# Symb0x76/ChineseChessZero

Hardware: AMD Instinct MI355X
Metric: self-play MCTS simulations/sec (higher is better)
Workload: dtype u8 rules / f32 Q (reference CPU path) / f64 PUCT (net: fp16)

## Files before the change

chinesechesszero_amd/_lib.py:

```python
from __future__ import annotations

import ctypes as C
import os

import torch

_HERE = os.path.dirname(os.path.abspath(__file__))
LIB_PATH = os.path.join(_HERE, "libcczero.so")

NSQ = 90
SQ_STRIDE = 96
NMOVES = 2086
MAX_LEGAL = 128
MASK_WORDS = 66
PLANES = 10710
REC_BYTES, REC_HDR, REC_IDS, REC_PI = 880, 96, 112, 368
REC_FLAGS, REC_FAST = 103, 1
REC_RESIGNED, REC_PLAYON, REC_VALUE = 2, 4, 8
REC_VALUE_OFF = 92
RESIGN_RESIGNED, RESIGN_PLAYON = 2, 4
HEAD_POL_STRIDE, HEAD_VAL_STRIDE = 1536, 640

ABI_VERSION = 9
CONV_RELU, CONV_DESCENDING, CONV_FORCE_SMALL, CONV_FORCE_TILE, CONV_G16, CONV_G16_EDGE_TILES = 1, 2, 16, 32, 64, 128
# ... 123 lines not shown
    "ccz_legal_moves": (C.c_int, [_P, C.c_int32, _P, _P, _P, _P, _P, _P]),
    "ccz_apply_moves": (C.c_int, [_P, C.c_int32, _P, _P, _P, _P]),
    "ccz_bias_act_f16": (C.c_int, [_P, _P, _P, _P, C.c_int64, C.c_int32]),
    "ccz_conv3x3_c256_f16": (C.c_int, [_P, _P, _P, _P, _P, _P, C.c_int64, C.c_int32]),
    "ccz_conv3x3_stem_f16": (C.c_int, [_P, _P, _P, _P, _P, C.c_int64, C.c_int32]),
    "ccz_pack_live_planes_f16": (C.c_int, [_P, _P, _P, C.c_int32]),
    "ccz_pack_live_planes_rows_f16": (C.c_int, [_P, _P, _P, C.c_int32, _P, _P]),
    "ccz_pack_live_planes_g16_f16": (C.c_int, [_P, _P, _P, C.c_int32, _P, _P]),
    "ccz_pack_conv_weights_g16_f16": (C.c_int, [_P, _P, _P, C.c_int32]),
    "ccz_conv3x3_c256_f16_live": (C.c_int, [_P, _P, _P, _P, _P, _P, C.c_int64, C.c_int32, _P, C.c_int32, C.c_int32]),
    "ccz_conv3x3_stem_f16_live": (C.c_int, [_P, _P, _P, _P, _P, C.c_int64, C.c_int32, _P, C.c_int32, C.c_int32]),
    "ccz_conv3x3_c256_heads_f16": (C.c_int, [_P, _P, _P, _P, _P, _P, _P, _P, _P, C.c_int64, C.c_int32, _P, C.c_int32, C.c_int32]),
    "ccz_heads_conv1x1_f16": (C.c_int, [_P, _P, _P, _P, _P, _P, C.c_int32, C.c_int32, _P]),
    "ccz_fc_f16": (C.c_int, [_P, _P, C.c_int32, _P, _P, _P, C.c_int32, C.c_int32, C.c_int32, C.c_int32, C.c_int32, _P]),
    "ccz_value_out_f32": (C.c_int, [_P, _P, _P, C.c_float, _P, C.c_int32, _P]),
}

_lib = None


def source_hash() -> str | None:
    import glob
    import hashlib
    csrc = os.path.join(_HERE, "csrc")
    files = sorted(glob.glob(os.path.join(csrc, "*.h")) + glob.glob(os.path.join(csrc, "*.hip")), key=os.path.basename)
    files.append(os.path.join(os.path.dirname(_HERE), "include", "cczero.h"))
    if len(files) < 2 or not all(os.path.exists(f) for f in files):
        return None
    h = hashlib.sha256()
    for f in files:
# ... 46 lines not shown
```

chinesechesszero_amd/build.py:

```python
from __future__ import annotations

import os
import subprocess

_HERE = os.path.dirname(os.path.abspath(__file__))


def build(verbose: bool = False) -> str:
    csrc = os.path.join(_HERE, "csrc")
    out = subprocess.run(["make", "-C", csrc], capture_output=True, text=True)
    if verbose or out.returncode != 0:
        print(out.stdout)
        print(out.stderr)
    if out.returncode != 0:
        raise RuntimeError("hipcc build of libcczero.so failed")
    path = os.path.join(_HERE, "libcczero.so")
    if not os.path.exists(path):
        raise RuntimeError("libcczero.so was not produced")
    return path


_HASHED = ("csrc/*.h", "csrc/*.hip", "csrc/Makefile", "engine.py", "selfplay.py", "net.py", "_lib.py", "replay.py", "../include/cczero.h", "../bench.py")


def code_hash() -> str:
# ... 10 lines not shown
```

chinesechesszero_amd/csrc/cczero.hip:

```cpp
#include "../../include/cczero.h"

#include <hip/hip_runtime.h>

#include <cmath>
#include <cstdarg>
#include <cstdio>
#include <cstring>
#include <new>
#include <vector>

#include "cczero_kernels.h"
#include "cczero_netops.h"
#include "cczero_conv.h"
#include "cczero_conv_small.h"
#include "cczero_conv_g16.h"
#include "cczero_conv_g16e.h"
#include "cczero_heads.h"

using namespace ccz;

namespace {

thread_local char g_err[512] = "";

// ... 37 lines not shown
    std::vector<void *> owned;
    size_t bytes = 0;
    int32_t *st_k = nullptr, *st_visits = nullptr, *st_rootn = nullptr;
    uint16_t *st_acts = nullptr;
    float *st_q = nullptr, *st_p = nullptr;
    double *st_pi = nullptr, *st_temps = nullptr;
    double *st_g = nullptr, *st_u = nullptr;
    long long *st_rowbase = nullptr;
    uint8_t *st_mask = nullptr, *st_sq = nullptr;
    std::vector<BoardMeta> h_meta;
    int active = 0;
    bool routed = false;
    uint8_t *route_red = nullptr;
    uint8_t *route_net = nullptr;
    uint64_t salt[2] = {0, 0};
    bool budgets_on = false;
    bool explore_on = false;
    uint8_t *proof = nullptr, *st_proof = nullptr;
    bool solver_on = false;
};

#define ACTIVE(e) ((unsigned)((e)->active > 0 ? (e)->active : (e)->d.B))

template <typename T> static int fetch_board_stats(ccz_engine *e, hipStream_t s, const T *dev, std::vector<T> &st)
{
    st.resize((size_t)e->d.B);
    HIP_TRY(hipMemcpyAsync(st.data(), dev, st.size() * sizeof(T), hipMemcpyDeviceToHost, s));
    HIP_TRY(hipStreamSynchronize(s));
    return 0;
}
// ... 151 lines not shown
    d.cache = nullptr;
    d.cache_mask = 0;
    if (cfg->eval_cache_log2) {
        const size_t slots = (size_t)1 << cfg->eval_cache_log2;
        d.cache_mask = (uint32_t)(slots - 1);
        ALLOC(d.cache, slots);
        ALLOC(d.claim, slots);
        ALLOC(d.cslot, B);
        ALLOC(d.ctag, B);
        ALLOC(d.cstate, B);
        ALLOC(d.cins, B);
        ALLOC(d.cver, B);
        ALLOC(d.crep, B);
        ALLOC(d.row_of, B);
        ALLOC(d.vleaf, B);
        if (he == hipSuccess) he = hipMemset(d.claim, 0x7f, slots * 4);
    }
    ALLOC(d.rec_sq, B * d.max_plies * 96);
    ALLOC(d.rec_turn, B * d.max_plies);
    ALLOC(d.rec_k, B * d.max_plies);
    ALLOC(d.rec_off, B * d.max_plies);
    ALLOC(d.rec_target, B * d.max_plies);
    ALLOC(d.budget, B);
    ALLOC(d.move_sims, B);
    ALLOC(d.target, B);
    ResignCfg *rs_cfg = nullptr;
    ALLOC(rs_cfg, 1);
    d.rs_cfg = rs_cfg;
    ALLOC(d.rs_state, B);
    ALLOC(d.rs_run, B * 2);
// ... 179 lines not shown
    hipStream_t s = (hipStream_t)stream;
    if (logits_f16)
        hipLaunchKernelGGL((k_softmax_gather<_Float16, false>), dim3(e->d.B), dim3(64), 0, s, e->d, (const _Float16 *)logits_dev, (const float *)nullptr);
    else
        hipLaunchKernelGGL((k_softmax_gather<float, false>), dim3(e->d.B), dim3(64), 0, s, e->d, (const float *)logits_dev, (const float *)nullptr);
    HIP_TRY(hipGetLastError());
    return 0;
}

int ccz_eval_plan(ccz_engine *e, void *stream, int32_t *miss_rows_dev, int32_t *n_miss_dev)
{
    NEED(e);
    if (!e->d.cache) return fail(-1, "ccz_eval_plan: the engine was created without an evaluation cache (ccz_config.eval_cache_log2)");
    if (!miss_rows_dev || !n_miss_dev) return fail(-1, "ccz_eval_plan: null output");
    hipStream_t s = (hipStream_t)stream;
    hipLaunchKernelGGL(k_cache_probe, dim3(e->d.B), dim3(64), 0, s, e->d);
    HIP_TRY(hipGetLastError());
    hipLaunchKernelGGL(k_cache_plan, dim3(1), dim3(1024), 0, s, e->d, miss_rows_dev, n_miss_dev);
    HIP_TRY(hipGetLastError());
    return 0;
}

int ccz_set_scouts(ccz_engine *e, int32_t n_scouts)
{
    NEED(e);
    if (n_scouts < 0 || n_scouts >= e->d.B) return fail(-1, "ccz_set_scouts: n_scouts must be in 0 .. n_boards - 1 (got %d of %d boards)", n_scouts, e->d.B);
    if (n_scouts && !e->d.cache) return fail(-1, "ccz_set_scouts: scouts work through the evaluation cache (ccz_config.eval_cache_log2)");
    if (n_scouts && e->budgets_on) return fail(-1, "ccz_set_scouts: not while simulation budgets are on (ccz_set_budgets(NULL) turns them off)");
    if (n_scouts && e->explore_on) return fail(-1, "ccz_set_scouts: not while root exploration is on (ccz_set_root_exploration)");
    e->active = n_scouts ? e->d.B - n_scouts : 0;
    return 0;
}

// ... 1044 lines not shown
    HIP_TRY(hipGetLastError());
    return 0;
}

int ccz_value_out_f32(void *stream, const void *h_dev, const void *w2_dev, float b2, float *v_dev, int32_t m, const int32_t *live_rows_dev)
{
    if (!h_dev || !w2_dev || !v_dev || m < 0) return fail(-1, "ccz_value_out_f32: bad arguments");
    if ((((uintptr_t)h_dev) | ((uintptr_t)w2_dev)) & 7) return fail(-1, "ccz_value_out_f32: h and w2 must be 8-byte aligned");
    if (m == 0) return 0;
    hipLaunchKernelGGL(k_value_out, dim3((unsigned)((m + 3) / 4)), dim3(256), 0, (hipStream_t)stream, (const _Float16 *)h_dev, (const _Float16 *)w2_dev, b2, v_dev,
                       (int)m, (const int *)live_rows_dev);
    HIP_TRY(hipGetLastError());
    return 0;
}

}
```

chinesechesszero_amd/csrc/cczero_heads.h:

```cpp
#pragma once
#include <hip/hip_runtime.h>
#include <stdint.h>

#include "cczero_conv.h"
#include "cczero_device.h"

namespace ccz {

constexpr int kHdPol = 17, kHdVal = 7;
constexpr int kHdPolStride = 1536;
constexpr int kHdValStride = 640;

template <bool G16>
__global__ __launch_bounds__(256) void k_head_conv1x1(const _Float16 *__restrict__ X, const _Float16 *__restrict__ Wh,
                                                        const float *__restrict__ bh, _Float16 *__restrict__ pol,
                                                        _Float16 *__restrict__ val, int n_boards, const int *__restrict__ live)
{
    const int lane = threadIdx.x & 63, r = lane & 15, q4 = lane >> 4;
    const int wave = blockIdx.x * 4 + (threadIdx.x >> 6), n_waves = gridDim.x * 4;
    int nb = n_boards;
    if (live) { const int l = *live; nb = l < nb ? l : nb; }
    const long n_rows = G16 ? (long)((nb + 15) >> 4) * 1440 : (long)nb * 90;
    const int n_cells = (int)((n_rows + 15) >> 4);
    if (wave >= n_cells) return;
// ... 55 lines not shown
            for (int s = 0; s < 8; ++s) b[s] = bn[s];
        }
    }
}

constexpr int kFcBM = 128, kFcBN = 128, kFcBK = 32, kFcStages = 4;
constexpr int kFcTile = 128 * kFcBK * 2;
constexpr int kFcStage = 2 * kFcTile;
constexpr int kFcERow = 144;
static_assert(4 * 64 * kFcERow <= kFcStages * kFcStage, "the epilogue blocks live in the operand ring");
#ifdef CCZ_FC_DIAG
#define FC_DBG(bit) (dbg & (bit))
#else
#define FC_DBG(bit) 0
#endif
template <bool RELU>
__global__ __launch_bounds__(256) void k_fc_f16(const _Float16 *__restrict__ A, int lda, const _Float16 *__restrict__ W,
                                                  const float *__restrict__ bias, _Float16 *__restrict__ C, int ldc, int M, int N,
                                                  int K, const int *__restrict__ live, [[maybe_unused]] int dbg)
{
    __shared__ __attribute__((aligned(16))) unsigned char lds[kFcStages * kFcStage];
    const int tid = threadIdx.x, lane = tid & 63, r = lane & 15, q4 = lane >> 4;
    const int wv = __builtin_amdgcn_readfirstlane(tid >> 6), wn = wv & 1, wm = wv >> 1;
    int Ml = M;
    if (live) { const int l = *live; Ml = l < Ml ? l : Ml; }
    const int mt = (Ml + kFcBM - 1) / kFcBM, nt = (N + kFcBN - 1) / kFcBN, tiles = mt * nt;
    int n0, m0;
    {
        const int b = blockIdx.x, x = b & 7, per = tiles >> 3, rem = tiles & 7;
        if ((b >> 3) >= per + (x < rem ? 1 : 0)) return;
        const int t = x * per + (x < rem ? x : rem) + (b >> 3);
        const int full = (mt >> 2) * 4 * nt;
        const int blk = t < full ? t / (4 * nt) : (mt >> 2);
        const int r_ = t < full ? t % (4 * nt) : t - full;
        const int cnt = t < full ? 4 : mt - 4 * blk;
        n0 = (r_ / cnt) * kFcBN;
        m0 = (4 * blk + r_ % cnt) * kFcBM;
    }
    const _Float16 *wsrc[2], *asrc[2];
    int wdst[2];
#pragma unroll
    for (int j = 0; j < 2; ++j) {
        const int row = (j * 4 + wv) * 16 + (lane >> 2), c = (lane & 3) ^ ((lane >> 4) & 3);
        wsrc[j] = W + (long)(n0 + row) * K + c * 8;
        int m = m0 + row;
        m = m < Ml ? m : Ml - 1;
        asrc[j] = A + (long)m * lda + c * 8;
        wdst[j] = (j * 4 + wv) * 1024;
    }
    auto issue = [&](int kt) {
        unsigned char *st = lds + (kt & (kFcStages - 1)) * kFcStage;
        const int k0 = kt * kFcBK;
        cv_glds16(wsrc[0] + k0, st + wdst[0]);
        cv_glds16(wsrc[1] + k0, st + wdst[1]);
        cv_glds16(asrc[0] + k0, st + kFcTile + wdst[0]);
        cv_glds16(asrc[1] + k0, st + kFcTile + wdst[1]);
    };
    cv_f32x4 acc[4][4];
#pragma unroll
    for (int i = 0; i < 4; ++i) {
        const float4 bv = *(const float4 *)(bias + n0 + wn * 64 + i * 16 + 4 * q4);
#pragma unroll
        for (int j = 0; j < 4; ++j) { acc[i][j][0] = bv.x; acc[i][j][1] = bv.y; acc[i][j][2] = bv.z; acc[i][j][3] = bv.w; }
    }
    const int nk = K / kFcBK;
    issue(0);
    if (nk > 1) issue(1);
    if (nk > 2) issue(2);
    const int foff = r * 64 + ((q4 ^ ((r >> 2) & 3)) << 4);
    for (int kt = 0; kt < nk; ++kt) {
        if (kt + 2 < nk) cv_wait_vm<8>();
        else if (kt + 1 < nk) cv_wait_vm<4>();
        else cv_wait_vm<0>();
        __builtin_amdgcn_sched_barrier(0);
        if (!FC_DBG(16)) __builtin_amdgcn_s_barrier();
        __builtin_amdgcn_sched_barrier(0);
        if (kt + 3 < nk && !FC_DBG(4)) issue(kt + 3);
        const unsigned char *wb = lds + (kt & (kFcStages - 1)) * kFcStage + wn * 4096 + foff;
        const unsigned char *ab = lds + (kt & (kFcStages - 1)) * kFcStage + kFcTile + wm * 4096 + foff;
        cv_half8 fa[4], fb[4];
        if (!FC_DBG(2) || kt == 0) {
#pragma unroll
            for (int i = 0; i < 4; ++i) fa[i] = *(const cv_half8 *)(wb + i * 1024);
#pragma unroll
            for (int j = 0; j < 4; ++j) fb[j] = *(const cv_half8 *)(ab + j * 1024);
        }
        if (!FC_DBG(1)) {
#pragma unroll
            for (int i = 0; i < 4; ++i)
#pragma unroll
                for (int j = 0; j < 4; ++j) acc[i][j] = __builtin_amdgcn_mfma_f32_16x16x32_f16(fa[i], fb[j], acc[i][j], 0, 0, 0);
        } else {
#pragma unroll
            for (int i = 0; i < 4; ++i) acc[i][0] += (cv_f32x4){(float)fa[i][0], (float)fb[i][0], 0.0f, 0.0f};
        }
    }
    if (FC_DBG(8)) { if (acc[0][0][0] == 12345.678f) C[0] = (_Float16)1; return; }
    __builtin_amdgcn_sched_barrier(0);
    __builtin_amdgcn_s_barrier();
    __builtin_amdgcn_sched_barrier(0);
    {
        unsigned char *tb = lds + wv * (64 * kFcERow);
#pragma unroll
        for (int j = 0; j < 4; ++j)
#pragma unroll
            for (int i = 0; i < 4; ++i) {
                float v0 = acc[i][j][0], v1 = acc[i][j][1], v2 = acc[i][j][2], v3 = acc[i][j][3];
                if (RELU) { v0 = fmaxf(v0, 0.0f); v1 = fmaxf(v1, 0.0f); v2 = fmaxf(v2, 0.0f); v3 = fmaxf(v3, 0.0f); }
                cv_half4 o;
                o[0] = (_Float16)v0; o[1] = (_Float16)v1; o[2] = (_Float16)v2; o[3] = (_Float16)v3;
                *(cv_half4 *)(tb + (j * 16 + r) * kFcERow + (i * 16 + 4 * q4) * 2) = o;
// ... 183 lines not shown
        }
    wave_sync();
    constexpr int NW = NF * 8;
#pragma unroll 4
    for (int it = 0; it < NW; ++it) {
        const int L = it * 64 + lane, row = L / NW, dw = L - row * NW;
        const int m = m0 + wm * 64 + row, n = n0 + I0 * 16 + 2 * dw;
        const uint32_t v = *(const uint32_t *)(tb + row * kFwERow + dw * 4);
        if (m < Ml && n + 1 < N) *(uint32_t *)(C + (long)m * ldc + n) = v;
    }
    FW_STAMP(3)
#undef FW_STAMP
}

template <bool RELU>
__global__ __launch_bounds__(512) void k_fc_wide_f16(const _Float16 *__restrict__ A, int lda, const _Float16 *__restrict__ W,
                                                       const float *__restrict__ bias, _Float16 *__restrict__ C, int ldc, int M, int N,
                                                       int K, const int *__restrict__ live, [[maybe_unused]] int dbg)
{
    __shared__ __attribute__((aligned(16))) unsigned char lds[kFwStages * kFwStage];
    const int tid = threadIdx.x, lane = tid & 63;
    const int wv = __builtin_amdgcn_readfirstlane(tid >> 6), wm = wv & 3, wn = wv >> 2;
    int Ml = M;
    if (live) { const int l = *live; Ml = l < Ml ? l : Ml; }
    const int mt = (Ml + kFwBM - 1) / kFwBM, nt = (N + kFwBN - 1) / kFwBN, tiles = mt * nt;
    int n0, m0;
    {
        const int b = blockIdx.x, x = b & 7, per = tiles >> 3, rem = tiles & 7;
        if ((b >> 3) >= per + (x < rem ? 1 : 0)) return;
        const int t = x * per + (x < rem ? x : rem) + (b >> 3);
        const int full = (mt >> 1) * 2 * nt;
        const int blk = t < full ? t / (2 * nt) : (mt >> 1);
        const int r_ = t < full ? t % (2 * nt) : t - full;
        const int cnt = t < full ? 2 : 1;
        n0 = (r_ / cnt) * kFwBN;
        m0 = (2 * blk + r_ % cnt) * kFwBM;
    }
    const int wrows = ((N + 127) >> 7) << 7;
    const int c = (lane & 7) ^ ((4 * (wv & 1) + (lane >> 4)) & 7), lr = lane >> 3;
    const _Float16 *src[7];
#pragma unroll
    for (int t = 0; t < 4; ++t) {
        int m = m0 + (wv + 8 * t) * 8 + lr;
        m = m < Ml ? m : Ml - 1;
        src[t] = A + (long)m * lda + c * 8;
    }
#pragma unroll
    for (int t = 0; t < 3; ++t) {
        int n = n0 + (wv + 8 * t) * 8 + lr;
        n = n < wrows ? n : wrows - 1;
        src[4 + t] = W + (long)n * K + c * 8;
    }
    if (wn == 0) fw_wave<RELU, 5, 0>(lds, src, wv, wm, lane, bias, wrows - 4, C, ldc, Ml, N, K, m0, n0, dbg);
    else fw_wave<RELU, 4, 5>(lds, src, wv, wm, lane, bias, wrows - 4, C, ldc, Ml, N, K, m0, n0, dbg);
}

__global__ __launch_bounds__(256) void k_value_out(const _Float16 *__restrict__ h, const _Float16 *__restrict__ w2, float b2,
                                                    float *__restrict__ v, int M, const int *__restrict__ live)
{
    const int lane = threadIdx.x & 63, m = blockIdx.x * 4 + (threadIdx.x >> 6);
    if (m >= M) return;
    const cv_half4 x = *(const cv_half4 *)(h + (long)m * 256 + lane * 4), w = *(const cv_half4 *)(w2 + lane * 4);
    int Ml = M;
    if (live) { const int l = *live; Ml = l < Ml ? l : Ml; }
    if (m >= Ml) return;
    float s = (float)x[0] * (float)w[0];
    s += (float)x[1] * (float)w[1];
    s += (float)x[2] * (float)w[2];
    s += (float)x[3] * (float)w[3];
    s = wave_sum_f32(s) + b2;
    if (lane == 0) v[m] = tanhf((float)(_Float16)s);
}

}
```

chinesechesszero_amd/csrc/cczero_kernels.h:

```cpp
#pragma once
#include <type_traits>

#include "cczero_device.h"

namespace ccz {

constexpr uint16_t kHalfOne = 0x3C00;
constexpr int kMaxDepth = 512;

__device__ __forceinline__ void set_err(const Dev &D, int bit) { atomicOr(D.err, bit); }

__device__ __forceinline__ int start_piece(int s)
{
    const int r = s / 9, f = s - 9 * r;
    const int rr = r <= 4 ? r : 9 - r;
    const int add = r <= 4 ? 0 : 8;
    int t = 0;
    if (rr == 0) {
        const int ff = f <= 4 ? f : 8 - f;
        t = ff == 0 ? ROOK : ff == 1 ? KNIGHT : ff == 2 ? BISHOP : ff == 3 ? ADVISOR : KING;
    } else if (rr == 2) {
        t = (f == 1 || f == 7) ? CANNON : 0;
    } else if (rr == 3) {
        t = (f & 1) ? 0 : PAWN;
// ... 1027 lines not shown
        }
    }
    if (tid == 0) {
        n_miss[0] = s_base[0];
        if (ROUTED) n_miss[1] = s_base[1];
    }
}

__global__ __launch_bounds__(1024) void k_cache_plan(Dev D, int32_t *miss_rows, int32_t *n_miss)
{
    __shared__ int s_wave[2][16];
    __shared__ int s_base[2];
    cache_plan_block<false>(D, miss_rows, n_miss, nullptr, 0ull, 0ull, s_wave, s_base);
}

__global__ __launch_bounds__(1024) void k_cache_plan_routed(Dev D, int32_t *miss_rows, int32_t *n_miss, const uint8_t *net, uint64_t salt0,
                                                            uint64_t salt1)
{
    __shared__ int s_wave[2][16];
    __shared__ int s_base[2];
    cache_plan_block<true>(D, miss_rows, n_miss, net, salt0, salt1, s_wave, s_base);
}

__device__ inline void plan_scouted_block(const Dev &D, int active, int32_t *miss_rows, int32_t *n_miss, int32_t *state_out, int tid, int nt, int &s_any)
{
    if (tid == 0) s_any = 0;
    __syncthreads();
    for (int b = tid; b < D.B; b += nt) {
        const int st = D.cstate[b];
        if (b < active) {
// ... 1180 lines not shown
```

chinesechesszero_amd/net.py:

```python
from __future__ import annotations

import ctypes as C
import os

import numpy as np
import torch
import torch.nn.functional as F
from torch import nn

PIECES = 7
PLAYS = 17


class ResBlock(nn.Module):

    def __init__(self, num_channels=256):
        super().__init__()
        self.conv1 = nn.Conv2d(num_channels, num_channels, kernel_size=(3, 3), stride=(1, 1), padding=1)
        self.conv1_bn = nn.BatchNorm2d(num_channels)
        self.conv1_act = nn.ReLU()
        self.conv2 = nn.Conv2d(num_channels, num_channels, kernel_size=(3, 3), stride=(1, 1), padding=1)
        self.conv2_bn = nn.BatchNorm2d(num_channels)
        self.conv2_act = nn.ReLU()

# ... 468 lines not shown
                         torch.zeros((Bx, _lib.HEAD_VAL_STRIDE), dtype=torch.float16, device=dev),
                         torch.empty((Bx, 256), dtype=torch.float16, device=dev))
        return bufs[key]

    def _heads_fused(self, x, B, g16, plan, conv_done=False):
        from . import _lib
        L = _lib.lib()
        Bx, dev = x.shape[0], x.device
        pol, val, h1 = self._head_buffers(Bx, dev)
        logits = torch.empty((B, 2086), dtype=torch.float16, device=dev)
        v = torch.empty((B,), dtype=torch.float32, device=dev)
        s = C.c_void_p(torch.cuda.current_stream(dev).cuda_stream)
        live = _ptr(plan[1]) if plan is not None else None
        if not conv_done:
            _lib.check(L.ccz_heads_conv1x1_f16(s, _ptr(x), _ptr(self.head_w32), _ptr(self.head_b32), _ptr(pol), _ptr(val), Bx, _lib.CONV_G16 if g16 else 0, live))
        _lib.check(L.ccz_fc_f16(s, _ptr(pol), _lib.HEAD_POL_STRIDE, _ptr(self.policy_fc_wp), _ptr(self.policy_fc_b32), _ptr(logits), 2086, B, 2086, 1536, 0, live))
        _lib.check(L.ccz_fc_f16(s, _ptr(val), _lib.HEAD_VAL_STRIDE, _ptr(self.value_fc1_wp), _ptr(self.value_fc1_b32), _ptr(h1), 256, B, 256, 640, 1, live))
        _lib.check(L.ccz_value_out_f32(s, _ptr(h1), _ptr(self.value_fc2_w), self._value_b2(), _ptr(v), B, live))
        return logits, v

    def _value_b2(self) -> float:
        b2 = self.__dict__.get("_b2")
        if b2 is None:
            b2 = self.__dict__["_b2"] = float(self.value_fc2_b.detach().float().cpu().item())
        return b2

    def _heads(self, x, B, g16, plan, return_logits, conv_done=False):
        if self._fused_heads_ok(x):
            logits, v = self._heads_fused(x, B, g16, plan, conv_done)
            if return_logits:
# ... 151 lines not shown
```

include/cczero.h:

```cpp
#ifndef CCZERO_H
#define CCZERO_H

#include <stdint.h>

#ifdef __cplusplus
extern "C" {
#endif

#define CCZ_ABI_VERSION 9
#define CCZ_NSQ 90
#define CCZ_SQ_STRIDE 96
#define CCZ_NMOVES 2086
#define CCZ_MAX_LEGAL 128
#define CCZ_MASK_WORDS 66
#define CCZ_PLANES 10710


#define CCZ_RULE_PAWN_MOVE_RESETS_CLOCK 2u
#define CCZ_RULE_PERPETUAL_CHECK 1u

#define CCZ_FLAG_REFERENCE_QUIRKS 1u
#define CCZ_FLAG_NO_MIRROR 2u
#define CCZ_FLAG_VALUE_F16 4u

// ... 232 lines not shown
                              const void *residual_dev, void *y_dev, int64_t n_pixels, int32_t relu,
                              const int32_t *live_rows_dev, int32_t part, int32_t n_parts);
int ccz_conv3x3_stem_f16_live(void *stream, const void *x64_dev, const void *w_dev, const void *bias_f32_dev,
                              void *y_dev, int64_t n_pixels, int32_t relu, const int32_t *live_rows_dev,
                              int32_t part, int32_t n_parts);

#define CCZ_HEAD_POL_STRIDE 1536
#define CCZ_HEAD_VAL_STRIDE 640
int ccz_heads_conv1x1_f16(void *stream, const void *x_dev, const void *w32_dev, const void *bias32_f32_dev, void *pol_dev,
                          void *val_dev, int32_t n_boards, int32_t flags, const int32_t *live_boards_dev);
int ccz_fc_f16(void *stream, const void *a_dev, int32_t lda, const void *w_dev, const void *bias_f32_dev, void *c_dev, int32_t ldc,
               int32_t m, int32_t n, int32_t k, int32_t relu, const int32_t *live_rows_dev);
int ccz_value_out_f32(void *stream, const void *h_dev, const void *w2_dev, float b2, float *v_dev, int32_t m,
                      const int32_t *live_rows_dev);

int ccz_conv3x3_c256_heads_f16(void *stream, const void *x_dev, const void *w_dev, const void *bias_f32_dev,
                               const void *residual_dev, const void *head_w32_dev, const void *head_bias32_f32_dev,
                               void *pol_dev, void *val_dev, int64_t n_pixels, int32_t flags,
                               const int32_t *live_rows_dev, int32_t part, int32_t n_parts);

#ifdef __cplusplus
}
#endif
#endif
```

profiles/summarize.py:

```python
#!/usr/bin/env python3
import csv
import glob
import json
import os
import sys
from collections import defaultdict


def find(d, pat):
    r = sorted(glob.glob(os.path.join(d, "**", pat), recursive=True))
    return r[0] if r else None


def main():
    out_dir, tag = sys.argv[1], sys.argv[2]
    root = os.path.dirname(os.path.abspath(__file__))
    summary = {}
    prev = os.path.join(root, f"{tag}_summary.json")
    if os.path.exists(prev):
        with open(prev) as f:
            summary = json.load(f)
    stats = find(os.path.join(out_dir, "trace"), "*kernel_stats.csv")
    if stats:
        rows = list(csv.DictReader(open(stats)))
        keep = rows[:48] + [r for r in rows[48:] if "ccz" in r.get("Name", "")]
        with open(os.path.join(root, f"{tag}_kernel_stats.csv"), "w", newline="") as f:
            w = csv.DictWriter(f, fieldnames=list(rows[0].keys()))
            w.writeheader()
            w.writerows(keep)
        for k in ("k_step", "k_softmax_gather", "k_select", "k_expand_backup", "k_finish_move", "k_harvest", "k_bias_act", "k_conv3x3"):
            hit = [r for r in rows if k in r.get("Name", "")]
            if hit:
                calls = sum(int(float(r.get("Calls", 0) or 0)) for r in hit)
                tot = sum(float(r.get("TotalDurationNs", 0) or 0) for r in hit)
                summary.setdefault(k, {})["avg_ns"] = tot / max(1, calls)
                summary[k]["calls"] = calls
                summary[k]["pct"] = sum(float(r.get("Percentage", 0) or 0) for r in hit)
                if len(hit) > 1:
                    summary[k]["variants"] = {r["Name"][:80]: {"calls": int(float(r["Calls"])), "avg_ns": float(r["AverageNs"])} for r in hit}
        plan_calls = sum(int(float(r.get("Calls", 0) or 0)) for r in rows if "k_cache_plan" in r.get("Name", ""))
        if plan_calls:
            tail = {}
            for k in ("k_cache_probe", "k_cache_plan", "k_pack_live_planes", "k_head_conv1x1", "k_fc_f16", "k_fc_wide_f16", "k_value_out", "k_softmax_gather"):
                tot = sum(float(r.get("TotalDurationNs", 0) or 0) for r in rows if k in r.get("Name", ""))
                calls = sum(int(float(r.get("Calls", 0) or 0)) for r in rows if k in r.get("Name", ""))
                if calls:
                    tail[k] = {"us_per_step": tot / plan_calls * 1e-3, "launches_per_step": calls / plan_calls, "avg_us": tot / calls * 1e-3}
            def fam(pred):
                hit = [r for r in rows if pred(r.get("Name", ""))]
                calls = sum(int(float(r.get("Calls", 0) or 0)) for r in hit)
                tot = sum(float(r.get("TotalDurationNs", 0) or 0) for r in hit)
                return calls, tot
            extra, detail = 0.0, {}
            for name, heads, plain in (("middle", lambda n: "k_conv3x3_g16_heads" in n, lambda n: "k_conv3x3_g16<true>" in n or "k_conv3x3_g16ILb1" in n),
                                       ("edge", lambda n: "k_conv3x3_g16_edge_heads" in n, lambda n: "k_conv3x3_g16_edge<true>" in n or "k_conv3x3_g16_edgeILb1" in n)):
                hc, ht = fam(heads)
                pc, pt = fam(plain)
                if hc and pc:
# ... 3 lines not shown
            if detail:
                tail["heads_in_last_tower_layer"] = {"us_per_step": extra, "launches_per_step": sum(v["launches_per_step"] for v in detail.values()),
                                                     "avg_us": extra / max(1e-9, sum(v["launches_per_step"] for v in detail.values())), "detail": detail,
                                                     "what": "launch time of the last layer with the heads in its epilogue minus an ordinary residual layer's, x launches per step "
                                                             "(the chains run concurrently: an upper bound on what the step pays)"}
            other = [(r.get("Name", ""), float(r.get("TotalDurationNs", 0) or 0), int(float(r.get("Calls", 0) or 0))) for r in rows
                     if "ccz" not in r.get("Name", "")]
            summary["evaluator_tail"] = {"kernels": tail, "us_per_step_ours": sum(v["us_per_step"] for v in tail.values()),
                                         "library_kernels_total_us_per_step": sum(t for _, t, _ in other) / plan_calls * 1e-3,
                                         "library_kernels_top": [{"name": n[:90], "us_per_step": t / plan_calls * 1e-3, "calls": c} for n, t, c in sorted(other, key=lambda x: -x[1])[:8]],
                                         "steps": plan_calls,
                                         "what": "non-tower evaluator work per lockstep step (rocprofv3 --kernel-trace --stats of bench.py --steps 120): cache probe + plan, "
                                                 "pack of the live planes, head convolutions, FC layers, value head, softmax + gather + cache store. "
                                                 "library_kernels_*: kernels that are not this library's (torch elementwise / GEMM / copies), whole run "
                                                 "(set-up, preroll and the CPU-side bookkeeping included) divided by the number of steps"}
    def bench_line(name):
        p = os.path.join(out_dir, name)
        if not os.path.exists(p):
            return None
        try:
            return json.loads([l for l in open(p).read().splitlines() if l.startswith("{")][-1])
        except Exception:
            return None

    both_here = all(find(os.path.join(out_dir, k), "*counter_collection.csv") for k in ("pmc_fetch", "pmc_write"))
    if both_here:
        for key in ("k_bar", "d_bar", "warning"):
            summary.get("k_step", {}).get("window", {}).pop(key, None)
    for kind, counter in (("pmc_fetch", "FETCH_SIZE"), ("pmc_write", "WRITE_SIZE"), ("pmc_cfetch", "FETCH_SIZE"), ("pmc_cwrite", "WRITE_SIZE"),
                          ("pmc_hfetch", "FETCH_SIZE"), ("pmc_hwrite", "WRITE_SIZE")):
# ... 112 lines not shown
```

Before: 200,000.

## Fuse cache probe and plan into one launch; fuse policy and value FC heads

Replaces the two-kernel cache probe plus single-block plan with one kernel that probes across many blocks and lets the last block to finish, detected through an atomic ticket, run the plan. It also adds a combined heads kernel for large batches: some workgroups compute the policy FC tile and others compute value FC1, ReLU and the value output using shared LDS. This removes launches and serialization at the step boundary. In exchange it adds the complexity of a last-block ticket and a heterogeneous grid.

```diff
diff --git a/chinesechesszero_amd/_lib.py b/chinesechesszero_amd/_lib.py
--- a/chinesechesszero_amd/_lib.py
+++ b/chinesechesszero_amd/_lib.py
@@ -161,6 +161,7 @@
     "ccz_heads_conv1x1_f16": (C.c_int, [_P, _P, _P, _P, _P, _P, C.c_int32, C.c_int32, _P]),
     "ccz_fc_f16": (C.c_int, [_P, _P, C.c_int32, _P, _P, _P, C.c_int32, C.c_int32, C.c_int32, C.c_int32, C.c_int32, _P]),
     "ccz_value_out_f32": (C.c_int, [_P, _P, _P, C.c_float, _P, C.c_int32, _P]),
+    "ccz_heads_fc_f16": (C.c_int, [_P, _P, _P, _P, _P, C.c_int32, _P, _P, _P, _P, C.c_float, _P, _P, C.c_int32, _P]),
 }
 
 _lib = None
diff --git a/chinesechesszero_amd/build.py b/chinesechesszero_amd/build.py
--- a/chinesechesszero_amd/build.py
+++ b/chinesechesszero_amd/build.py
@@ -8,7 +8,7 @@
 
 def build(verbose: bool = False) -> str:
     csrc = os.path.join(_HERE, "csrc")
-    out = subprocess.run(["make", "-C", csrc], capture_output=True, text=True)
+    out = subprocess.run(["make", "-j2", "-C", csrc, "all", "twolaunch"], capture_output=True, text=True)
     if verbose or out.returncode != 0:
         print(out.stdout)
         print(out.stderr)
diff --git a/chinesechesszero_amd/csrc/cczero.hip b/chinesechesszero_amd/csrc/cczero.hip
--- a/chinesechesszero_amd/csrc/cczero.hip
+++ b/chinesechesszero_amd/csrc/cczero.hip
@@ -75,6 +75,7 @@
     uint8_t *route_red = nullptr;
     uint8_t *route_net = nullptr;
     uint64_t salt[2] = {0, 0};
+    uint32_t *plan_ticket = nullptr;
     bool budgets_on = false;
     bool explore_on = false;
     uint8_t *proof = nullptr, *st_proof = nullptr;
@@ -256,6 +257,7 @@
         ALLOC(d.crep, B);
         ALLOC(d.row_of, B);
         ALLOC(d.vleaf, B);
+        ALLOC(e->plan_ticket, 1);
         if (he == hipSuccess) he = hipMemset(d.claim, 0x7f, slots * 4);
     }
     ALLOC(d.rec_sq, B * d.max_plies * 96);
@@ -465,9 +467,13 @@
     if (!e->d.cache) return fail(-1, "ccz_eval_plan: the engine was created without an evaluation cache (ccz_config.eval_cache_log2)");
     if (!miss_rows_dev || !n_miss_dev) return fail(-1, "ccz_eval_plan: null output");
     hipStream_t s = (hipStream_t)stream;
+#ifdef CCZ_EVAL_PLAN_TWO_LAUNCH
     hipLaunchKernelGGL(k_cache_probe, dim3(e->d.B), dim3(64), 0, s, e->d);
     HIP_TRY(hipGetLastError());
     hipLaunchKernelGGL(k_cache_plan, dim3(1), dim3(1024), 0, s, e->d, miss_rows_dev, n_miss_dev);
+#else
+    hipLaunchKernelGGL(k_eval_plan, dim3((unsigned)((e->d.B + kPlanWaves - 1) / kPlanWaves)), dim3(64 * kPlanWaves), 0, s, e->d, miss_rows_dev, n_miss_dev, e->plan_ticket);
+#endif
     HIP_TRY(hipGetLastError());
     return 0;
 }
@@ -1542,4 +1548,23 @@
     return 0;
 }
 
-}
+int ccz_heads_fc_f16(void *stream, const void *pol_dev, const void *wp_dev, const void *bp_f32_dev, void *logits_dev, int32_t ldc, const void *val_dev,
+                     const void *w1_dev, const void *b1_f32_dev, const void *w2_dev, float b2, float *v_dev, void *h1_dev, int32_t m, const int32_t *live_rows_dev)
+{
+    constexpr int n = 2086;
+    if (!pol_dev || !wp_dev || !bp_f32_dev || !logits_dev || !val_dev || !w1_dev || !b1_f32_dev || !w2_dev || !v_dev || m < 0) return fail(-1, "ccz_heads_fc_f16: bad arguments");
+    if ((ldc & 1) || ldc < n) return fail(-1, "ccz_heads_fc_f16: ldc must be even and >= %d", n);
+    if ((((uintptr_t)pol_dev) | ((uintptr_t)wp_dev) | ((uintptr_t)bp_f32_dev) | ((uintptr_t)val_dev) | ((uintptr_t)w1_dev) | ((uintptr_t)b1_f32_dev)) & 15 ||
+        ((uintptr_t)logits_dev & 3) || ((uintptr_t)w2_dev & 7) || ((uintptr_t)v_dev & 3) || ((uintptr_t)h1_dev & 7))
+        return fail(-1, "ccz_heads_fc_f16: pol, val, the FC weights and biases must be 16-byte aligned, w2 and h1 8-byte, logits and v 4-byte aligned");
+    if (m == 0) return 0;
+    const int wtiles = ((n + kFwBN - 1) / kFwBN) * ((m + kFwBM - 1) / kFwBM);
+    const int pol_blocks = 8 * ((wtiles + 7) / 8), val_blocks = (m + kHvTiles * kFcBM - 1) / (kHvTiles * kFcBM);
+    hipLaunchKernelGGL(k_heads_fc_f16, dim3((unsigned)(pol_blocks + val_blocks)), dim3(512), 0, (hipStream_t)stream, (const _Float16 *)pol_dev, (const _Float16 *)wp_dev,
+                       (const float *)bp_f32_dev, (_Float16 *)logits_dev, (int)ldc, n, (const _Float16 *)val_dev, (const _Float16 *)w1_dev, (const float *)b1_f32_dev,
+                       (const _Float16 *)w2_dev, b2, v_dev, (_Float16 *)h1_dev, (int)m, (const int *)live_rows_dev, pol_blocks, (int)kHdPolStride);
+    HIP_TRY(hipGetLastError());
+    return 0;
+}
+
+}
diff --git a/chinesechesszero_amd/csrc/cczero_heads.h b/chinesechesszero_amd/csrc/cczero_heads.h
--- a/chinesechesszero_amd/csrc/cczero_heads.h
+++ b/chinesechesszero_amd/csrc/cczero_heads.h
@@ -93,6 +93,70 @@
 #else
 #define FC_DBG(bit) 0
 #endif
+__device__ __forceinline__ void fc_tile_acc(unsigned char *lds, const _Float16 *__restrict__ A, int lda, const _Float16 *__restrict__ W,
+                                            const float *__restrict__ bias, int Ml, int K, int m0, int n0, int wv, int lane,
+                                            cv_f32x4 (&acc)[4][4], [[maybe_unused]] int dbg)
+{
+    const int r = lane & 15, q4 = lane >> 4, wn = wv & 1, wm = wv >> 1;
+    const _Float16 *wsrc[2], *asrc[2];
+    int wdst[2];
+#pragma unroll
+    for (int j = 0; j < 2; ++j) {
+        const int row = (j * 4 + wv) * 16 + (lane >> 2), c = (lane & 3) ^ ((lane >> 4) & 3);
+        wsrc[j] = W + (long)(n0 + row) * K + c * 8;
+        int m = m0 + row;
+        m = m < Ml ? m : Ml - 1;
+        asrc[j] = A + (long)m * lda + c * 8;
+        wdst[j] = (j * 4 + wv) * 1024;
+    }
+    auto issue = [&](int kt) {
+        unsigned char *st = lds + (kt & (kFcStages - 1)) * kFcStage;
+        const int k0 = kt * kFcBK;
+        cv_glds16(wsrc[0] + k0, st + wdst[0]);
+        cv_glds16(wsrc[1] + k0, st + wdst[1]);
+        cv_glds16(asrc[0] + k0, st + kFcTile + wdst[0]);
+        cv_glds16(asrc[1] + k0, st + kFcTile + wdst[1]);
+    };
+#pragma unroll
+    for (int i = 0; i < 4; ++i) {
+        const float4 bv = *(const float4 *)(bias + n0 + wn * 64 + i * 16 + 4 * q4);
+#pragma unroll
+        for (int j = 0; j < 4; ++j) { acc[i][j][0] = bv.x; acc[i][j][1] = bv.y; acc[i][j][2] = bv.z; acc[i][j][3] = bv.w; }
+    }
+    const int nk = K / kFcBK;
+    issue(0);
+    if (nk > 1) issue(1);
+    if (nk > 2) issue(2);
+    const int foff = r * 64 + ((q4 ^ ((r >> 2) & 3)) << 4);
+    for (int kt = 0; kt < nk; ++kt) {
+        if (kt + 2 < nk) cv_wait_vm<8>();
+        else if (kt + 1 < nk) cv_wait_vm<4>();
+        else cv_wait_vm<0>();
+        __builtin_amdgcn_sched_barrier(0);
+        if (!FC_DBG(16)) __builtin_amdgcn_s_barrier();
+        __builtin_amdgcn_sched_barrier(0);
+        if (kt + 3 < nk && !FC_DBG(4)) issue(kt + 3);
+        const unsigned char *wb = lds + (kt & (kFcStages - 1)) * kFcStage + wn * 4096 + foff;
+        const unsigned char *ab = lds + (kt & (kFcStages - 1)) * kFcStage + kFcTile + wm * 4096 + foff;
+        cv_half8 fa[4], fb[4];
+        if (!FC_DBG(2) || kt == 0) {
+#pragma unroll
+            for (int i = 0; i < 4; ++i) fa[i] = *(const cv_half8 *)(wb + i * 1024);
+#pragma unroll
+            for (int j = 0; j < 4; ++j) fb[j] = *(const cv_half8 *)(ab + j * 1024);
+        }
+        if (!FC_DBG(1)) {
+#pragma unroll
+            for (int i = 0; i < 4; ++i)
+#pragma unroll
+                for (int j = 0; j < 4; ++j) acc[i][j] = __builtin_amdgcn_mfma_f32_16x16x32_f16(fa[i], fb[j], acc[i][j], 0, 0, 0);
+        } else {
+#pragma unroll
+            for (int i = 0; i < 4; ++i) acc[i][0] += (cv_f32x4){(float)fa[i][0], (float)fb[i][0], 0.0f, 0.0f};
+        }
+    }
+}
+
 template <bool RELU>
 __global__ __launch_bounds__(256) void k_fc_f16(const _Float16 *__restrict__ A, int lda, const _Float16 *__restrict__ W,
                                                   const float *__restrict__ bias, _Float16 *__restrict__ C, int ldc, int M, int N,
@@ -116,64 +180,8 @@
         n0 = (r_ / cnt) * kFcBN;
         m0 = (4 * blk + r_ % cnt) * kFcBM;
     }
-    const _Float16 *wsrc[2], *asrc[2];
-    int wdst[2];
-#pragma unroll
-    for (int j = 0; j < 2; ++j) {
-        const int row = (j * 4 + wv) * 16 + (lane >> 2), c = (lane & 3) ^ ((lane >> 4) & 3);
-        wsrc[j] = W + (long)(n0 + row) * K + c * 8;
-        int m = m0 + row;
-        m = m < Ml ? m : Ml - 1;
-        asrc[j] = A + (long)m * lda + c * 8;
-        wdst[j] = (j * 4 + wv) * 1024;
-    }
-    auto issue = [&](int kt) {
-        unsigned char *st = lds + (kt & (kFcStages - 1)) * kFcStage;
-        const int k0 = kt * kFcBK;
-        cv_glds16(wsrc[0] + k0, st + wdst[0]);
-        cv_glds16(wsrc[1] + k0, st + wdst[1]);
-        cv_glds16(asrc[0] + k0, st + kFcTile + wdst[0]);
-        cv_glds16(asrc[1] + k0, st + kFcTile + wdst[1]);
-    };
     cv_f32x4 acc[4][4];
-#pragma unroll
-    for (int i = 0; i < 4; ++i) {
-        const float4 bv = *(const float4 *)(bias + n0 + wn * 64 + i * 16 + 4 * q4);
-#pragma unroll
-        for (int j = 0; j < 4; ++j) { acc[i][j][0] = bv.x; acc[i][j][1] = bv.y; acc[i][j][2] = bv.z; acc[i][j][3] = bv.w; }
-    }
-    const int nk = K / kFcBK;
-    issue(0);
-    if (nk > 1) issue(1);
-    if (nk > 2) issue(2);
-    const int foff = r * 64 + ((q4 ^ ((r >> 2) & 3)) << 4);
-    for (int kt = 0; kt < nk; ++kt) {
-        if (kt + 2 < nk) cv_wait_vm<8>();
-        else if (kt + 1 < nk) cv_wait_vm<4>();
-        else cv_wait_vm<0>();
-        __builtin_amdgcn_sched_barrier(0);
-        if (!FC_DBG(16)) __builtin_amdgcn_s_barrier();
-        __builtin_amdgcn_sched_barrier(0);
-        if (kt + 3 < nk && !FC_DBG(4)) issue(kt + 3);
-        const unsigned char *wb = lds + (kt & (kFcStages - 1)) * kFcStage + wn * 4096 + foff;
-        const unsigned char *ab = lds + (kt & (kFcStages - 1)) * kFcStage + kFcTile + wm * 4096 + foff;
-        cv_half8 fa[4], fb[4];
-        if (!FC_DBG(2) || kt == 0) {
-#pragma unroll
-            for (int i = 0; i < 4; ++i) fa[i] = *(const cv_half8 *)(wb + i * 1024);
-#pragma unroll
-            for (int j = 0; j < 4; ++j) fb[j] = *(const cv_half8 *)(ab + j * 1024);
-        }
-        if (!FC_DBG(1)) {
-#pragma unroll
-            for (int i = 0; i < 4; ++i)
-#pragma unroll
-                for (int j = 0; j < 4; ++j) acc[i][j] = __builtin_amdgcn_mfma_f32_16x16x32_f16(fa[i], fb[j], acc[i][j], 0, 0, 0);
-        } else {
-#pragma unroll
-            for (int i = 0; i < 4; ++i) acc[i][0] += (cv_f32x4){(float)fa[i][0], (float)fb[i][0], 0.0f, 0.0f};
-        }
-    }
+    fc_tile_acc(lds, A, lda, W, bias, Ml, K, m0, n0, wv, lane, acc, dbg);
     if (FC_DBG(8)) { if (acc[0][0][0] == 12345.678f) C[0] = (_Float16)1; return; }
     __builtin_amdgcn_sched_barrier(0);
     __builtin_amdgcn_s_barrier();
@@ -387,19 +395,16 @@
 }
 
 template <bool RELU>
-__global__ __launch_bounds__(512) void k_fc_wide_f16(const _Float16 *__restrict__ A, int lda, const _Float16 *__restrict__ W,
-                                                       const float *__restrict__ bias, _Float16 *__restrict__ C, int ldc, int M, int N,
-                                                       int K, const int *__restrict__ live, [[maybe_unused]] int dbg)
-{
-    __shared__ __attribute__((aligned(16))) unsigned char lds[kFwStages * kFwStage];
+__device__ __forceinline__ void fw_block(unsigned char *lds, int b, const _Float16 *__restrict__ A, int lda, const _Float16 *__restrict__ W,
+                                         const float *__restrict__ bias, _Float16 *__restrict__ C, int ldc, int Ml, int N, int K,
+                                         [[maybe_unused]] int dbg)
+{
     const int tid = threadIdx.x, lane = tid & 63;
     const int wv = __builtin_amdgcn_readfirstlane(tid >> 6), wm = wv & 3, wn = wv >> 2;
-    int Ml = M;
-    if (live) { const int l = *live; Ml = l < Ml ? l : Ml; }
     const int mt = (Ml + kFwBM - 1) / kFwBM, nt = (N + kFwBN - 1) / kFwBN, tiles = mt * nt;
     int n0, m0;
     {
-        const int b = blockIdx.x, x = b & 7, per = tiles >> 3, rem = tiles & 7;
+        const int x = b & 7, per = tiles >> 3, rem = tiles & 7;
         if ((b >> 3) >= per + (x < rem ? 1 : 0)) return;
         const int t = x * per + (x < rem ? x : rem) + (b >> 3);
         const int full = (mt >> 1) * 2 * nt;
@@ -428,6 +433,27 @@
     else fw_wave<RELU, 4, 5>(lds, src, wv, wm, lane, bias, wrows - 4, C, ldc, Ml, N, K, m0, n0, dbg);
 }
 
+template <bool RELU>
+__global__ __launch_bounds__(512) void k_fc_wide_f16(const _Float16 *__restrict__ A, int lda, const _Float16 *__restrict__ W,
+                                                       const float *__restrict__ bias, _Float16 *__restrict__ C, int ldc, int M, int N,
+                                                       int K, const int *__restrict__ live, [[maybe_unused]] int dbg)
+{
+    __shared__ __attribute__((aligned(16))) unsigned char lds[kFwStages * kFwStage];
+    int Ml = M;
+    if (live) { const int l = *live; Ml = l < Ml ? l : Ml; }
+    fw_block<RELU>(lds, blockIdx.x, A, lda, W, bias, C, ldc, Ml, N, K, dbg);
+}
+
+__device__ __forceinline__ float value_out_wave(cv_half4 x, cv_half4 w, float b2)
+{
+    float s = (float)x[0] * (float)w[0];
+    s += (float)x[1] * (float)w[1];
+    s += (float)x[2] * (float)w[2];
+    s += (float)x[3] * (float)w[3];
+    s = wave_sum_f32(s) + b2;
+    return tanhf((float)(_Float16)s);
+}
+
 __global__ __launch_bounds__(256) void k_value_out(const _Float16 *__restrict__ h, const _Float16 *__restrict__ w2, float b2,
                                                     float *__restrict__ v, int M, const int *__restrict__ live)
 {
@@ -437,12 +463,62 @@
     int Ml = M;
     if (live) { const int l = *live; Ml = l < Ml ? l : Ml; }
     if (m >= Ml) return;
-    float s = (float)x[0] * (float)w[0];
-    s += (float)x[1] * (float)w[1];
-    s += (float)x[2] * (float)w[2];
-    s += (float)x[3] * (float)w[3];
-    s = wave_sum_f32(s) + b2;
-    if (lane == 0) v[m] = tanhf((float)(_Float16)s);
-}
-
-}
+    const float t = value_out_wave(x, w, b2);
+    if (lane == 0) v[m] = t;
+}
+
+constexpr int kHvK = 640, kHvHidden = 256;
+constexpr int kHvHRow = kHvHidden * 2 + 16;
+constexpr int kHvTiles = 2;
+static_assert(2 * kFcStages * kFcStage <= kFwStages * kFwStage && kFcBM * kHvHRow <= kFwStages * kFwStage, "the value workgroup lives in the policy tile's LDS");
+
+__device__ __forceinline__ void hv_block(unsigned char *lds, int vb, const _Float16 *__restrict__ A, const _Float16 *__restrict__ W1,
+                                         const float *__restrict__ b1, const _Float16 *__restrict__ w2, float b2, float *__restrict__ v, _Float16 *__restrict__ h1, int Ml)
+{
+    const int tid = threadIdx.x, lane = tid & 63, r = lane & 15, q4 = lane >> 4;
+    const int wv = __builtin_amdgcn_readfirstlane(tid >> 6), half = wv >> 2, w4 = wv & 3, wn = w4 & 1, wm = w4 >> 1;
+    const int n0 = half * kFcBN;
+    const cv_half4 w = *(const cv_half4 *)(w2 + lane * 4);
+    for (int t = 0; t < kHvTiles; ++t) {
+        const int m0 = (vb * kHvTiles + t) * kFcBM;
+        if (m0 >= Ml) return;
+        cv_f32x4 acc[4][4];
+        fc_tile_acc(lds + half * (kFcStages * kFcStage), A, kHdValStride, W1, b1, Ml, kHvK, m0, n0, w4, lane, acc, 0);
+        __syncthreads();
+#pragma unroll
+        for (int j = 0; j < 4; ++j)
+#pragma unroll
+            for (int i = 0; i < 4; ++i) {
+                cv_half4 o;
+                o[0] = (_Float16)fmaxf(acc[i][j][0], 0.0f); o[1] = (_Float16)fmaxf(acc[i][j][1], 0.0f);
+                o[2] = (_Float16)fmaxf(acc[i][j][2], 0.0f); o[3] = (_Float16)fmaxf(acc[i][j][3], 0.0f);
+                *(cv_half4 *)(lds + (wm * 64 + j * 16 + r) * kHvHRow + (n0 + wn * 64 + i * 16 + 4 * q4) * 2) = o;
+            }
+        __syncthreads();
+        for (int it = 0; it < kFcBM / 8; ++it) {
+            const int row = wv * (kFcBM / 8) + it, m = m0 + row;
+            if (m >= Ml) break;
+            const cv_half4 x = *(const cv_half4 *)(lds + row * kHvHRow + lane * 8);
+            if (h1) *(cv_half4 *)(h1 + (long)m * kHvHidden + lane * 4) = x;
+            const float y = value_out_wave(x, w, b2);
+            if (lane == 0) v[m] = y;
+        }
+        __syncthreads();
+    }
+}
+
+__global__ __launch_bounds__(512) void k_heads_fc_f16(const _Float16 *__restrict__ pol, const _Float16 *__restrict__ Wp, const float *__restrict__ bp,
+                                                        _Float16 *__restrict__ C, int ldc, int N, const _Float16 *__restrict__ val,
+                                                        const _Float16 *__restrict__ W1, const float *__restrict__ b1,
+                                                        const _Float16 *__restrict__ w2, float b2, float *__restrict__ v, _Float16 *__restrict__ h1, int M,
+                                                        const int *__restrict__ live, int pol_blocks, int Kp)
+{
+    __shared__ __attribute__((aligned(16))) unsigned char lds[kFwStages * kFwStage];
+    int Ml = M;
+    if (live) { const int l = *live; Ml = l < Ml ? l : Ml; }
+    const int b = blockIdx.x;
+    if (b < pol_blocks) fw_block<false>(lds, b, pol, Kp, Wp, bp, C, ldc, Ml, N, Kp, 0);
+    else hv_block(lds, b - pol_blocks, val, W1, b1, w2, b2, v, h1, Ml);
+}
+
+}
diff --git a/chinesechesszero_amd/csrc/cczero_kernels.h b/chinesechesszero_amd/csrc/cczero_kernels.h
--- a/chinesechesszero_amd/csrc/cczero_kernels.h
+++ b/chinesechesszero_amd/csrc/cczero_kernels.h
@@ -1065,6 +1065,30 @@
     cache_plan_block<false>(D, miss_rows, n_miss, nullptr, 0ull, 0ull, s_wave, s_base);
 }
 
+constexpr int kPlanWaves = 16;
+__global__ __launch_bounds__(64 * kPlanWaves) void k_eval_plan(Dev D, int32_t *miss_rows, int32_t *n_miss, uint32_t *ticket)
+{
+    __shared__ int s_wave[2][16];
+    __shared__ int s_base[2];
+    __shared__ int s_last;
+    const int tid = threadIdx.x;
+    const int b = blockIdx.x * kPlanWaves + __builtin_amdgcn_readfirstlane(tid >> 6);
+    if (b < D.B) (void)cache_probe_wave(D, b, tid & 63);
+    __syncthreads();
+    if (tid == 0) {
+        __threadfence();
+        const bool last = __hip_atomic_fetch_add(ticket, 1u, __ATOMIC_RELAXED, __HIP_MEMORY_SCOPE_AGENT) == gridDim.x - 1u;
+        if (last) {
+            __threadfence();
+            __hip_atomic_store(ticket, 0u, __ATOMIC_RELAXED, __HIP_MEMORY_SCOPE_AGENT);
+        }
+        s_last = last;
+    }
+    __syncthreads();
+    if (!s_last) return;
+    cache_plan_block<false>(D, miss_rows, n_miss, nullptr, 0ull, 0ull, s_wave, s_base);
+}
+
 __global__ __launch_bounds__(1024) void k_cache_plan_routed(Dev D, int32_t *miss_rows, int32_t *n_miss, const uint8_t *net, uint64_t salt0,
                                                             uint64_t salt1)
 {
diff --git a/chinesechesszero_amd/net.py b/chinesechesszero_amd/net.py
--- a/chinesechesszero_amd/net.py
+++ b/chinesechesszero_amd/net.py
@@ -506,6 +506,10 @@
         live = _ptr(plan[1]) if plan is not None else None
         if not conv_done:
             _lib.check(L.ccz_heads_conv1x1_f16(s, _ptr(x), _ptr(self.head_w32), _ptr(self.head_b32), _ptr(pol), _ptr(val), Bx, _lib.CONV_G16 if g16 else 0, live))
+        if B >= 2048 and hasattr(L, "ccz_heads_fc_f16"):
+            _lib.check(L.ccz_heads_fc_f16(s, _ptr(pol), _ptr(self.policy_fc_wp), _ptr(self.policy_fc_b32), _ptr(logits), 2086, _ptr(val),
+                                          _ptr(self.value_fc1_wp), _ptr(self.value_fc1_b32), _ptr(self.value_fc2_w), self._value_b2(), _ptr(v), _ptr(h1), B, live))
+            return logits, v
         _lib.check(L.ccz_fc_f16(s, _ptr(pol), _lib.HEAD_POL_STRIDE, _ptr(self.policy_fc_wp), _ptr(self.policy_fc_b32), _ptr(logits), 2086, B, 2086, 1536, 0, live))
         _lib.check(L.ccz_fc_f16(s, _ptr(val), _lib.HEAD_VAL_STRIDE, _ptr(self.value_fc1_wp), _ptr(self.value_fc1_b32), _ptr(h1), 256, B, 256, 640, 1, live))
         _lib.check(L.ccz_value_out_f32(s, _ptr(h1), _ptr(self.value_fc2_w), self._value_b2(), _ptr(v), B, live))
diff --git a/include/cczero.h b/include/cczero.h
--- a/include/cczero.h
+++ b/include/cczero.h
@@ -270,6 +270,10 @@
 int ccz_value_out_f32(void *stream, const void *h_dev, const void *w2_dev, float b2, float *v_dev, int32_t m,
                       const int32_t *live_rows_dev);
 
+int ccz_heads_fc_f16(void *stream, const void *pol_dev, const void *wp_dev, const void *bp_f32_dev, void *logits_dev, int32_t ldc,
+                     const void *val_dev, const void *w1_dev, const void *b1_f32_dev, const void *w2_dev, float b2, float *v_dev,
+                     void *h1_dev, int32_t m, const int32_t *live_rows_dev);
+
 int ccz_conv3x3_c256_heads_f16(void *stream, const void *x_dev, const void *w_dev, const void *bias_f32_dev,
                                const void *residual_dev, const void *head_w32_dev, const void *head_bias32_f32_dev,
                                void *pol_dev, void *val_dev, int64_t n_pixels, int32_t flags,
diff --git a/profiles/summarize.py b/profiles/summarize.py
--- a/profiles/summarize.py
+++ b/profiles/summarize.py
@@ -12,7 +12,53 @@
     return r[0] if r else None
 
 
+TAIL_KERNELS = ("k_cache_probe", "k_cache_plan", "k_eval_plan", "k_pack_live_planes", "k_head_conv1x1", "k_fc_f16", "k_fc_wide_f16", "k_heads_fc_f16", "k_value_out",
+                "k_softmax_gather", "k_step")
+
+
+def is_plan(name):
+    return ("k_eval_plan" in name or "k_cache_plan" in name) and "routed" not in name and "scouted" not in name
+
+
+def step_boundary(trace_csv):
+    rows = []
+    with open(trace_csv) as f:
+        for r in csv.DictReader(f):
+            rows.append((int(r["Start_Timestamp"]), int(r["End_Timestamp"]), r["Kernel_Name"]))
+    rows.sort()
+    gaps, busy, inside, conv_end, seen_other = [], defaultdict(float), [], None, False
+    for st, en, name in rows:
+        if "k_conv3x3" in name:
+            if conv_end is not None and seen_other:
+                names = [n for _, _, n in inside]
+                if any(is_plan(n) for n in names) and not any("k_finish_move" in n for n in names):
+                    gaps.append((st - conv_end) * 1e-3)
+                    for a, b, n in inside:
+                        for k in TAIL_KERNELS:
+                            if k in n:
+                                busy[k] += (b - a) * 1e-3
+                                break
+                        else:
+                            busy["other"] += (b - a) * 1e-3
+            conv_end = max(conv_end, en) if conv_end is not None and not seen_other else en
+            seen_other, inside = False, []
+        elif conv_end is not None:
+            seen_other = True
+            inside.append((st, en, name))
+    if not gaps:
+        return None
+    g = sorted(gaps)
+    q = lambda p: g[min(len(g) - 1, int(p * len(g)))]
+    return {"boundaries": len(g), "median_us": q(0.5), "p10_us": q(0.1), "p90_us": q(0.9), "mean_us": sum(g) / len(g),
+            "kernel_busy_us_per_boundary": {k: v / len(g) for k, v in sorted(busy.items())},
+            "what": "GPU time from the end of a step's last k_conv3x3* kernel to the start of the next step's first k_conv3x3* kernel, over the "
+                    "boundaries in which the plan kernel ran and k_finish_move did not (rocprofv3 --kernel-trace of bench.py --steps 120)"}
+
+
 def main():
+    if sys.argv[1] == "--boundary":
+        print(json.dumps(step_boundary(sys.argv[2]), indent=1))
+        return
     out_dir, tag = sys.argv[1], sys.argv[2]
     root = os.path.dirname(os.path.abspath(__file__))
     summary = {}
@@ -38,10 +84,10 @@
                 summary[k]["pct"] = sum(float(r.get("Percentage", 0) or 0) for r in hit)
                 if len(hit) > 1:
                     summary[k]["variants"] = {r["Name"][:80]: {"calls": int(float(r["Calls"])), "avg_ns": float(r["AverageNs"])} for r in hit}
-        plan_calls = sum(int(float(r.get("Calls", 0) or 0)) for r in rows if "k_cache_plan" in r.get("Name", ""))
+        plan_calls = sum(int(float(r.get("Calls", 0) or 0)) for r in rows if is_plan(r.get("Name", "")))
         if plan_calls:
             tail = {}
-            for k in ("k_cache_probe", "k_cache_plan", "k_pack_live_planes", "k_head_conv1x1", "k_fc_f16", "k_fc_wide_f16", "k_value_out", "k_softmax_gather"):
+            for k in TAIL_KERNELS[:-1]:
                 tot = sum(float(r.get("TotalDurationNs", 0) or 0) for r in rows if k in r.get("Name", ""))
                 calls = sum(int(float(r.get("Calls", 0) or 0)) for r in rows if k in r.get("Name", ""))
                 if calls:
@@ -75,6 +121,12 @@
                                                  "pack of the live planes, head convolutions, FC layers, value head, softmax + gather + cache store. "
                                                  "library_kernels_*: kernels that are not this library's (torch elementwise / GEMM / copies), whole run "
                                                  "(set-up, preroll and the CPU-side bookkeeping included) divided by the number of steps"}
+    trace_csv = find(os.path.join(out_dir, "trace"), "*kernel_trace.csv")
+    if trace_csv:
+        gap = step_boundary(trace_csv)
+        if gap:
+            summary["step_boundary_gap"] = gap
+
     def bench_line(name):
         p = os.path.join(out_dir, name)
         if not os.path.exists(p):
```

After: 199,500. Within noise of the previous version (-0.3%).
